# synnada-ai/datafusion-upstream

Measured on AMD Instinct MI355X. Metric: rows/sec hash-join+agg, TPC-H SF100 Q3, higher is better.
Workload: dtype int64; 1 GPU; TPC-H SF100 Q3 (3-way hash join + group-by SUM + sort), int64 keys, Decimal128(15,2) money, resident in HBM; input_rows=765043119, parallelism=1 GPU

## Files before the change

datafusion-upstream_amd/csrc/core.hip:

```cpp
#include "device_utils.h"
#include <mutex>

namespace dfgpu {

void fail(dfgpu_status code, const char* fmt, ...) {
  char buf[1024]; va_list ap; va_start(ap, fmt); vsnprintf(buf, sizeof buf, fmt, ap); va_end(ap);
  throw Error(code, buf);
}

struct CtxRefs { std::atomic<int64_t> n{1}; };
static std::mutex g_mu;
static std::vector<std::pair<dfgpu_ctx*, CtxRefs*>> g_ctx;
static CtxRefs* refs_of(dfgpu_ctx* c) { std::lock_guard<std::mutex> l(g_mu); for (auto& p : g_ctx) if (p.first == c) return p.second; return nullptr; }
static void ctx_unref(dfgpu_ctx* c) {
  CtxRefs* r = refs_of(c);
  if (!r || r->n.fetch_sub(1) != 1) return;
  { std::lock_guard<std::mutex> l(g_mu); for (size_t i = 0; i < g_ctx.size(); i++) if (g_ctx[i].first == c) { g_ctx.erase(g_ctx.begin() + i); break; } }
  (void)hipSetDevice(c->device);
  (void)hipStreamSynchronize(c->stream);
  if (c->free_blocks) { for (auto& b : *c->free_blocks) (void)hipFree(b.second); delete c->free_blocks; }
  delete c->alloc_mu;
  if (c->d_flags) (void)hipFree(c->d_flags);
  if (c->d_scratch64) (void)hipFree(c->d_scratch64);
  if (c->h_pinned) (void)hipHostFree(c->h_pinned);
  for (auto& sp : c->spans) if (sp.start) { (void)hipEventDestroy(sp.start); (void)hipEventDestroy(sp.stop); }
  if (c->copy_stream) { (void)hipStreamSynchronize(c->copy_stream); (void)hipStreamDestroy(c->copy_stream); }
  if (c->own_stream) (void)hipStreamDestroy(c->stream);
  delete r; delete c;
}

static size_t size_class(size_t bytes) {
  size_t n = 256;
  while (n < bytes) { size_t m = n + n / 2; if (m >= bytes && n >= 512) return m; n <<= 1; }
  return n;
}
Buffer::~Buffer() {
  if (owned && ptr && ctx) {
    { std::lock_guard<std::mutex> l(*ctx->alloc_mu); ctx->free_blocks->emplace_back(bytes, ptr); ctx->cached_bytes += bytes; ctx->live_bytes -= bytes; }
// ... 52 lines not shown
  struct Restore { dfgpu_ctx* c; int v; ~Restore() { c->defer_flag_checks = v; } } r{ctx, saved};
  check_flags(ctx, what.c_str());
}
void check_flags(dfgpu_ctx* ctx, const char* what) {
  if (ctx->defer_flag_checks > 0) { if (!ctx->flags_pending) ctx->flags_what = what; else if (ctx->flags_what.find(what) == std::string::npos) ctx->flags_what += std::string(", ") + what; ctx->flags_pending = true; return; }
  uint32_t f = 0;
  ctx->count_sync((std::string("sync:flags:") + what).c_str());
  fetch_to_pinned(ctx, 63, ctx->d_flags, 4);
  f = *(uint32_t*)(ctx->h_pinned + 63);
  if (!f) return;
  HIP_CHECK(hipMemsetAsync(ctx->d_flags, 0, 4, ctx->stream));
  if (f & DFGPU_FLAG_DIV_ZERO) fail(DFGPU_EXECUTION, "Arrow error: Divide by zero error (%s)", what);
  if (f & DFGPU_FLAG_OVERFLOW) fail(DFGPU_EXECUTION, "Arrow error: Arithmetic overflow (%s)", what);
  if (f & DFGPU_FLAG_CAST) fail(DFGPU_EXECUTION, "Arrow error: Cast error: value out of range (%s)", what);
  if (f & DFGPU_FLAG_OOB) fail(DFGPU_EXECUTION, "Arrow error: index out of bounds (%s)", what);
  if (f & DFGPU_FLAG_STALLED) fail(DFGPU_INTERNAL, "a workgroup gave up waiting for the tile counts of the workgroups in front of it; the result of that sort is not valid (%s; option sort_onesweep_rows=0 selects the three-launch passes)", what);
  fail(DFGPU_INTERNAL, "kernel raised flag %u (%s)", f, what);
}
__global__ void __launch_bounds__(512) k_post_words(const uint32_t* src, int nwords, uint32_t* h_dst, unsigned long long* h_seq, unsigned long long seq) {
  const int i = threadIdx.x;
  if (i < nwords) __hip_atomic_store(h_dst + i, src[i], __ATOMIC_RELAXED, __HIP_MEMORY_SCOPE_SYSTEM);
  __threadfence_system();
  __syncthreads();
  if (i == 0) __hip_atomic_store(h_seq, seq, __ATOMIC_RELEASE, __HIP_MEMORY_SCOPE_SYSTEM);
}
void fetch_to_pinned(dfgpu_ctx* ctx, int h_word, const void* d_src, size_t bytes) {
  if (bytes == 0 || (bytes & 3) || h_word < 0 || (size_t)h_word * 8 + bytes > (size_t)dfgpu_ctx::MAIL_WORDS * 8) fail(DFGPU_INTERNAL, "fetch_to_pinned: %zu bytes at word %d", bytes, h_word);
  if (!ctx->mailbox_readback) {
    HIP_CHECK(hipMemcpyAsync(ctx->h_pinned + h_word, d_src, bytes, hipMemcpyDeviceToHost, ctx->stream));
    HIP_CHECK(hipStreamSynchronize(ctx->stream));
    return;
// ... 269 lines not shown
  { "agg_partitioned_force", OPT_BOOL(agg_partitioned_force) },
  { "agg_partitioned_min_rows", OPT_INT(agg_partitioned_min_rows) },
  { "agg_pack_estimate_min_rows", OPT_INT(agg_pack_estimate_min_rows) },
  { "agg_preaggregate_distinct", OPT_READ(pa_last_distinct) },
  { "agg_spill_state_bytes", OPT_INT(agg_spill_state_bytes) },
  { "agg_spill_ranges", OPT_RANGE(agg_spill_ranges, 1, 4096) },
  { "sort_packed_keys", OPT_BOOL(sort_packed_keys) },
  { "sort_packed_min_rows", OPT_MIN(sort_packed_min_rows, 2) },
  { "sort_estimate_ranges", OPT_BOOL(sort_estimate_ranges) },
  { "sort_topk_words_min_rows", OPT_MIN(sort_topk_words_min_rows, 2) },
  { "sort_one_block_max_rows", OPT_MIN(sort_one_block_max_rows, 0) },
  { "sort_onesweep_min_rows", OPT_MIN(sort_onesweep_min_rows, 2) },
  { "sort_onesweep_rows", OPT_GET(sort_onesweep_rows), [](dfgpu_ctx* c, int64_t v) { c->sort_onesweep_rows = v == 16 ? 16 : v > 0 ? 8 : 0; } },
  { "sort_onesweep_fused_finish", OPT_BOOL(sort_onesweep_fused_finish) },
  { "sort_fused_small_passes", OPT_BOOL(sort_fused_small_passes) },
  { "sort_spill_bytes", OPT_INT(sort_spill_bytes) },
  { "sort_spill_ranges", OPT_RANGE(sort_spill_ranges, 1, 4096) },
  { "spm_merge_rows", OPT_GET(spm_merge_rows), [](dfgpu_ctx* c, int64_t v) { if (v < 0) fail(DFGPU_INVALID_ARGUMENT, "spm_merge_rows: >= 0"); c->spm_merge_rows = v; } },
  { "memory_limit", OPT_INT(memory_limit) },
  { "live_bytes", OPT_READ(live_bytes) },
  { "cached_bytes", OPT_READ(cached_bytes) },
  { "trim_cache", nullptr, [](dfgpu_ctx* c, int64_t) {
      HIP_CHECK(hipStreamSynchronize(c->stream));
      std::lock_guard<std::mutex> l(*c->alloc_mu); for (auto& x : *c->free_blocks) (void)hipFree(x.second); c->free_blocks->clear(); c->cached_bytes = 0; } },
  { "mailbox_readback", OPT_BOOL(mailbox_readback) },
  { "collect_metrics", OPT_BOOL(collect_metrics) },
  { "defer_flag_checks", OPT_GET(defer_flag_checks), [](dfgpu_ctx* c, int64_t v) {
      if (v) c->defer_flag_checks++;
      else { if (c->defer_flag_checks > 0) c->defer_flag_checks--; if (c->defer_flag_checks == 0) flush_flags(c); } } },
};
// ... 410 lines not shown
```

datafusion-upstream_amd/csrc/device_utils.h:

```cpp
#pragma once
#include "dfgpu_internal.h"

namespace dfgpu {

using i128 = __int128;
using u128 = unsigned __int128;

constexpr int WAVE = 64;
constexpr int BLOCK = 256;

__host__ __device__ inline uint64_t mix64(uint64_t x) {
  x += 0x9e3779b97f4a7c15ULL;
  x = (x ^ (x >> 30)) * 0xbf58476d1ce4e5b9ULL;
  x = (x ^ (x >> 27)) * 0x94d049bb133111ebULL;
  return x ^ (x >> 31);
}
__host__ __device__ inline uint64_t combine_hashes(uint64_t l, uint64_t r) { return ((uint64_t)(17 * 37) + l) * 37 + r; }

__device__ inline bool bit_get(const uint64_t* w, int64_t i) { return (w[i >> 6] >> (i & 63)) & 1; }
__device__ inline bool valid_at(const uint64_t* w, int64_t i) { return w == nullptr || bit_get(w, i); }

__device__ inline int lane_id() { return threadIdx.x & 63; }
__device__ inline uint64_t lanemask_lt() { return (1ull << lane_id()) - 1ull; }
__device__ inline uint64_t ballot64(bool p) { return __ballot(p); }
// ... 6 lines not shown
#pragma unroll
  for (int d = 32; d > 0; d >>= 1) v += __shfl_xor(v, d, 64);
  return v;
}
template <typename T> __device__ inline T block_exclusive_sum(T v, T* lds, T* total) {
  T inc = wave_inclusive_sum(v);
  int w = threadIdx.x >> 6;
  __syncthreads();
  if (lane_id() == 63) lds[w] = inc;
  __syncthreads();
  T base = 0, tot = 0;
#pragma unroll
  for (int i = 0; i < BLOCK / WAVE; i++) { T x = lds[i]; if (i < w) base += x; tot += x; }
  *total = tot;
  return base + inc - v;
}

__device__ inline int64_t key_at(const void* keys, int32_t key_type, int64_t i) {
  switch (key_type) {
    case DFGPU_INT8: return ((const int8_t*)keys)[i];
    case DFGPU_INT16: return ((const int16_t*)keys)[i];
    case DFGPU_INT32: case DFGPU_DATE32: return ((const int32_t*)keys)[i];
    case DFGPU_INT64: return ((const int64_t*)keys)[i];
    case DFGPU_UINT8: return ((const uint8_t*)keys)[i];
    case DFGPU_UINT16: return ((const uint16_t*)keys)[i];
    case DFGPU_UINT32: return ((const uint32_t*)keys)[i];
    default: return (int64_t)((const uint64_t*)keys)[i];
  }
}
__device__ inline bool cell_resolve(const ColView& c, int64_t i, int64_t* row) {
// ... 68 lines not shown
```

datafusion-upstream_amd/csrc/dfgpu_internal.h:

```cpp
#pragma once
#include <hip/hip_runtime.h>
#include <atomic>
#include <cstdarg>
#include <cstdint>
#include <cstdio>
#include <cstring>
#include <memory>
#include <mutex>
#include <stdexcept>
#include <string>
#include <vector>
#include "../../include/dfgpu.h"

namespace dfgpu {

struct Error : std::exception {
  dfgpu_status code; std::string msg;
  Error(dfgpu_status c, std::string m) : code(c), msg(std::move(m)) {}
  const char* what() const noexcept override { return msg.c_str(); }
};
[[noreturn]] void fail(dfgpu_status code, const char* fmt, ...);

#define HIP_CHECK(expr)                                                                         \
  do { hipError_t e_ = (expr);                                                                  \
// ... 41 lines not shown
  uint32_t* d_flags = nullptr;
  uint64_t* d_scratch64 = nullptr;
  uint64_t* h_pinned = nullptr;
  static constexpr int MAIL_SEQ = 384, MAIL_WORDS = 256, PINNED_WORDS = 512;
  bool mailbox_readback = true; uint64_t mail_seq = 0;
  int num_cus = 256;
  std::mutex* alloc_mu = nullptr;
  std::vector<std::pair<size_t, void*>>* free_blocks = nullptr;
  size_t cached_bytes = 0, live_bytes = 0;
  int64_t sort_packed_min_rows = 1 << 20;
  int64_t sort_topk_words_min_rows = 1 << 23;
  int64_t sort_one_block_max_rows = 8192;
  int64_t sort_onesweep_min_rows = 1 << 20;
  bool sort_onesweep_fused_finish = true;
  int sort_onesweep_rows = 16;
  bool sort_fused_small_passes = true;
  bool sort_estimate_ranges = true;
  int64_t spm_merge_rows = (int64_t)1 << 25;
  int64_t sort_spill_bytes = 0, sort_spill_ranges = 16;
  int64_t agg_spill_state_bytes = 0, agg_spill_ranges = 16;
  int64_t memory_limit = 0;
  bool collect_metrics = false;
  struct Span { hipEvent_t start = nullptr, stop = nullptr; };
  std::vector<Span> spans;
  std::mutex span_mu;
  bool profile = false; std::string profile_only;
  std::vector<std::pair<std::string, int64_t>> sync_counts;
  void count_sync(const char* why) { if (!profile) return; for (auto& kv : sync_counts) if (kv.first == why) { kv.second++; return; } sync_counts.emplace_back(why, 1); }
  struct ProfRec { const char* name; hipEvent_t start, stop; };
  std::vector<ProfRec> prof;
// ... 88 lines not shown
struct KeySet { int32_t n; ColView c[MAX_KEYS]; };
struct DenseCol { const void* keys; const uint64_t* key_valid; const uint32_t* canon; const uint64_t* dict_valid; int64_t dict_len; uint32_t n_ids, stride; int32_t key_type; };
struct DenseCols { int32_t n; DenseCol c[MAX_KEYS]; };
struct DeferredIds {
  int kind = 0;
  DenseCols dc{}; int32_t key_type = 0; BufferPtr mask, dense_map; std::vector<BufferPtr> keep;
  BufferPtr heads, prefix; uint32_t base = 0;
};
void materialize_ids(dfgpu_ctx* ctx, const dfgpu_array* ids);
KeySet make_keyset(const dfgpu_array* const* cols, int32_t n);

BufferPtr effective_mask(dfgpu_ctx* ctx, const dfgpu_array* mask, int64_t expect_len);

void exclusive_scan_u32(dfgpu_ctx* ctx, const uint32_t* in, uint64_t* out, int64_t n, uint64_t* d_total );
void exclusive_scan_u32_inplace32(dfgpu_ctx* ctx, uint32_t* data, int64_t n, uint64_t* d_total);

dfgpu_array* take_impl(dfgpu_ctx* ctx, const dfgpu_array* values, const void* idx, int idx_width, const uint64_t* idx_validity, int64_t n_out);
dfgpu_array* mask_to_indices_impl(dfgpu_ctx* ctx, const uint64_t* bits, int64_t n);
dfgpu_array* mask_to_indices_checked(dfgpu_ctx* ctx, const uint64_t* bits, int64_t n, int check_slot, uint64_t* check_value);
dfgpu_array* mask_to_indices_uncounted(dfgpu_ctx* ctx, const uint64_t* bits, int64_t n, uint64_t* d_count = nullptr);
int64_t count_set_bits(dfgpu_ctx* ctx, const uint64_t* bits, int64_t n);
inline const uint64_t* row_selection_words(dfgpu_ctx* ctx, int64_t n) { return ctx->row_selection && ctx->row_selection_len == n ? (const uint64_t*)ctx->row_selection->ptr : nullptr; }

void launch_iota_u32(dfgpu_ctx* ctx, uint32_t* out, int64_t n, uint32_t start);
void launch_set_bits_prefix(dfgpu_ctx* ctx, uint64_t* bits, int64_t m);

void hash_keys_device(dfgpu_ctx* ctx, const dfgpu_array* const* cols, int32_t k, uint64_t seed, uint64_t* out);

void radix_sort_pairs_u32(dfgpu_ctx* ctx, uint32_t* keys, uint32_t* vals, int64_t n, int bits);

struct KernelTimer {
  dfgpu_ctx* c; int idx = -1;
  KernelTimer(dfgpu_ctx* ctx, const char* name) : c(ctx) {
    if (!c->profile || (!c->profile_only.empty() && c->profile_only != name)) return;
// ... 25 lines not shown
```

datafusion-upstream_amd/csrc/groups.hip:

```cpp
#include "device_utils.h"
#include <algorithm>

namespace dfgpu {
constexpr uint64_t G_EMPTY = ~0ull;
constexpr uint32_t G_NEW = 0x80000000u;
constexpr uint32_t G_NONE = 0xFFFFFFFFu;
constexpr uint64_t GROUP_SEED = 0x5851f42d4c957f2dULL;
}
using namespace dfgpu;

enum class GroupRep : uint8_t { NONE, RUNS, PRIMITIVE, DENSE, DIRECT_MAP, HASHED };

struct dfgpu_groups {
  dfgpu_ctx* ctx = nullptr; int32_t nkeys = 0;
  int64_t n_groups = 0;
  GroupRep rep = GroupRep::NONE;
  std::vector<dfgpu_array*> keys;
  int64_t size_hint = 0;
  std::vector<dfgpu_array*> lazy_src; dfgpu_array* lazy_rows = nullptr;
  BufferPtr pslots; uint64_t pcap = 0; bool prim_banned = false;
  uint64_t capacity = 0; BufferPtr slots, first_row;
  BufferPtr ghash; int64_t ghash_cap = 0;
  bool canon_mode = false;
  struct Canon { dfgpu_array* dict = nullptr; BufferPtr ids; int64_t n_ids = 0; };
// ... 475 lines not shown
  if (!ctx->group_run_detection || ctx->force_hash_collisions || mk || g->capacity != 0 || !(g->n_groups == 0 || g->rep == GroupRep::RUNS) || !run_key_type(k0) ||
      (g->n_groups && logical_type(k0) != g->keys[0]->type)) return false;
  KernelTimer kt_(ctx, "k_groups_runs");
  BufferPtr heads = alloc_buffer(ctx, bitmap_bytes(n));
  zero_scratch(ctx);
  int w = type_width(k0->type);
  const void* prev = g->n_groups ? (const void*)((const char*)g->keys[0]->values->ptr + (size_t)(g->n_groups - 1) * w) : nullptr;
  dim3 grid(grid_for(n, BLOCK)), block(BLOCK);
#define RUNS(T) do { if (nkeys == 1) hipLaunchKernelGGL((k_run_heads1<T>), dim3(grid_for(n, BLOCK * 4)), block, 0, ctx->stream, (const T*)k0->values->ptr, n, (const T*)prev, (uint64_t*)heads->ptr, (unsigned long long*)(ctx->d_scratch64 + 2)); \
                     else hipLaunchKernelGGL((k_run_heads<T>), grid, block, 0, ctx->stream, bk, n, (const T*)prev, (uint64_t*)heads->ptr, (unsigned long long*)(ctx->d_scratch64 + 2)); } while (0)
  switch (k0->type) {
    case DFGPU_INT8: RUNS(int8_t); break; case DFGPU_INT16: RUNS(int16_t); break; case DFGPU_INT32: case DFGPU_DATE32: RUNS(int32_t); break; case DFGPU_INT64: RUNS(int64_t); break;
    case DFGPU_UINT8: RUNS(uint8_t); break; case DFGPU_UINT16: RUNS(uint16_t); break; case DFGPU_UINT32: RUNS(uint32_t); break; default: RUNS(uint64_t); break; }
#undef RUNS
  KERNEL_CHECK();
  ArrayHolder firsts(mask_to_indices_checked(ctx, (const uint64_t*)heads->ptr, n, 2, nullptr));
  if (!firsts.get()) return false;
  int64_t n_new = firsts.get()->length;
  if (g->n_groups + n_new >= (int64_t)G_NEW) fail(DFGPU_RESOURCES_EXHAUSTED, "more than 2^31 groups");
  int64_t nw = (n + 63) / 64;
  BufferPtr prefix = alloc_buffer(ctx, (size_t)nw * 4);
  hipLaunchKernelGGL(k_popc_words_g, dim3(grid_for(nw, BLOCK)), block, 0, ctx->stream, (const uint64_t*)heads->ptr, nw, (uint32_t*)prefix->ptr);
  exclusive_scan_u32_inplace32(ctx, (uint32_t*)prefix->ptr, nw, nullptr);
  if (allow_deferred && n >= (1 << 20)) {
    auto d = std::make_shared<DeferredIds>(); d->kind = 1; d->heads = heads; d->prefix = prefix; d->base = (uint32_t)g->n_groups; ids->deferred_ids = d;
  } else hipLaunchKernelGGL(k_run_ids, grid, block, 0, ctx->stream, (const uint64_t*)heads->ptr, (const uint32_t*)prefix->ptr, n, (uint32_t)g->n_groups, (uint32_t*)ids->values->ptr);
  KERNEL_CHECK();
  if (n_new && g->n_groups == 0 && ctx->group_lazy_keys && n_new >= (1 << 16)) {
    for (int c = 0; c < nkeys; c++) { g->lazy_src.push_back(const_cast<dfgpu_array*>(cols[c])); dfgpu_array_retain(g->lazy_src.back()); }
    g->lazy_rows = firsts.release();
  } else if (n_new) groups_append_keys(ctx, g, cols, nkeys, firsts.get(), n_new);
  g->n_groups += n_new; g->rep = GroupRep::RUNS;
  return true;
}
static bool prim_key_type(const dfgpu_array* a) { return a && (a->type == DFGPU_INT64 || a->type == DFGPU_UINT64 || a->type == DFGPU_INT32 || a->type == DFGPU_UINT32 || a->type == DFGPU_DATE32) && !a->validity; }
static void prim_rebuild(dfgpu_ctx* ctx, dfgpu_groups* g, uint64_t cap, bool key4) {
  g->pslots = alloc_buffer(ctx, (size_t)cap * sizeof(PSlot)); g->pcap = cap; HIP_CHECK(hipMemsetAsync(g->pslots->ptr, 0xFF, (size_t)cap * sizeof(PSlot), ctx->stream));
  if (!g->n_groups) return;
// ... 285 lines not shown
```

datafusion-upstream_amd/csrc/join.hip:

```cpp
#include "join_table.h"

namespace dfgpu {
constexpr uint64_t SLOT_EMPTY = ~0ull;
constexpr uint32_t NO_SLOT = 0xFFFFFFFFu;
}
using namespace dfgpu;


namespace dfgpu {

__device__ inline bool row_selected(const uint64_t* mask, int64_t i) { return mask == nullptr || bit_get(mask, i); }

__global__ void __launch_bounds__(BLOCK) k_join_build(KeySet ks, int64_t n, const uint64_t* mask, int null_eq, int force_zero,
                                                      uint64_t* slots, uint32_t* slot_count, uint64_t cap_mask, uint32_t* row_slot,
                                                      unsigned long long* counters ) {
  int64_t i = (int64_t)blockIdx.x * BLOCK + threadIdx.x;
  if (i >= n) return;
  uint32_t my_slot = NO_SLOT;
  if (row_selected(mask, i)) {
    bool any_null; uint64_t h = keyset_hash(ks, i, 0, &any_null);
    if (force_zero) h = 0;
    if (!any_null || null_eq) {
      uint64_t tag = h >> 32, s = h & cap_mask, mine = (tag << 32) | (uint64_t)i;
      for (uint64_t step = 0; step <= cap_mask; step++) {
// ... 568 lines not shown
  else {
    t->bitmap = alloc_buffer(ctx, bitmap_bytes((int64_t)range)); t->mem += (int64_t)bitmap_bytes((int64_t)range);
    HIP_CHECK(hipMemsetAsync(t->bitmap->ptr, t->rank_identity ? 0xFF : 0, bitmap_bytes((int64_t)range), ctx->stream));
  }
  if (!t->rank_identity) {
    if (mk && !runs && n <= 0xFFFFFFF0ll) {
      t->sel_rows = mask_to_indices_uncounted(ctx, mk, n, ctx->d_scratch64 + 15); t->mem += t->sel_rows->length * 4;
      DFGPU_INT_KEY_DISPATCH(key0->type, hipLaunchKernelGGL((k_key_setbits_rows<T>), dim3(grid_for(n, BLOCK, ctx->num_cus * 16)), dim3(BLOCK), 0, ctx->stream, (const T*)kv, (const uint32_t*)t->sel_rows->values->ptr,
                                                            (const unsigned long long*)(ctx->d_scratch64 + 15), (int64_t)lo, (uint64_t*)t->bitmap->ptr));
    } else {
      DFGPU_INT_KEY_DISPATCH(key0->type, hipLaunchKernelGGL((k_key_setbits_masked<T>), dim3(grid_for(n, BLOCK)), dim3(BLOCK), 0, ctx->stream, (const T*)kv, mk, n, (int64_t)lo, (uint64_t*)t->bitmap->ptr));
      if (mk) { t->sel_rows = mask_to_indices_impl(ctx, mk, n); t->mem += t->sel_rows->length * 4; }
    }
    KERNEL_CHECK();
    t->rank_prefix = alloc_buffer(ctx, (size_t)nw * 4);
    hipLaunchKernelGGL(k_popc_words, dim3(grid_for(nw, BLOCK)), dim3(BLOCK), 0, ctx->stream, (const uint64_t*)t->bitmap->ptr, nw, (uint32_t*)t->rank_prefix->ptr);
    exclusive_scan_u32_inplace32(ctx, (uint32_t*)t->rank_prefix->ptr, nw, nullptr);
    KERNEL_CHECK();
    t->mem += nw * 4;
  }
  return true;
}

template <typename T>
__global__ void __launch_bounds__(BLOCK) k_key_minmax_masked(const T* keys, const uint64_t* valid, const uint64_t* mask, int64_t n, long long* mn, long long* mx, const uint32_t* rows = nullptr, const unsigned long long* d_count = nullptr) {
  long long lo = INT64_MAX, hi = INT64_MIN;
  if (rows) {
    const int64_t m = (int64_t)*d_count;
    for (int64_t j = (int64_t)blockIdx.x * BLOCK + threadIdx.x; j < m; j += (int64_t)gridDim.x * BLOCK) { const int64_t i = rows[j]; if (valid_at(valid, i)) { long long v = (long long)keys[i]; lo = v < lo ? v : lo; hi = v > hi ? v : hi; } }
  } else
  for (int64_t i = (int64_t)blockIdx.x * BLOCK + threadIdx.x; i < n; i += (int64_t)gridDim.x * BLOCK)
    if (row_selected(mask, i) && valid_at(valid, i)) { long long v = (long long)keys[i]; lo = v < lo ? v : lo; hi = v > hi ? v : hi; }
// ... 45 lines not shown
      DFGPU_INT_KEY_DISPATCH(key0->type, hipLaunchKernelGGL((k_key_gather_minmax<T>), dim3(grid_for(n, BLOCK * 4, ctx->num_cus * 4)), dim3(BLOCK), 0, ctx->stream, (const T*)key0->values->ptr, rl, dcount, (T*)ck->ptr,
                                                            w, w + 1)); });
    lo = mm[0]; hi = mm[1];
  } else selected_key_range(ctx, t, "sync:rank_index_range", &lo, &hi);
  t->have_minmax = true; t->sel_min = lo; t->sel_max = hi;
  if (lo > hi) return false;
  const uint64_t range = (uint64_t)hi - (uint64_t)lo + 1;
  if (range == 0 || range > (1ull << 32) || range > (uint64_t)n * 256 + 65536) return false;
  const int64_t nw = (int64_t)((range + 63) / 64);
  BufferPtr bitmap = alloc_buffer(ctx, bitmap_bytes((int64_t)range));
  HIP_CHECK(hipMemsetAsync(bitmap->ptr, 0, bitmap_bytes((int64_t)range), ctx->stream));
  HIP_CHECK(hipMemsetAsync(ctx->d_scratch64 + 6, 0, 8, ctx->stream));
  DFGPU_INT_KEY_DISPATCH(key0->type, hipLaunchKernelGGL((k_key_setbits_unique<T>), dim3(lgrid), dim3(BLOCK), 0, ctx->stream, (const T*)key0->values->ptr, mk, rl, dcount, n, (int64_t)lo, (uint64_t*)bitmap->ptr,
                                                        (unsigned long long*)(ctx->d_scratch64 + 6), (const T*)ckp));
  BufferPtr prefix = alloc_buffer(ctx, (size_t)nw * 4);
  hipLaunchKernelGGL(k_popc_words, dim3(grid_for(nw, BLOCK)), dim3(BLOCK), 0, ctx->stream, (const uint64_t*)bitmap->ptr, nw, (uint32_t*)prefix->ptr);
  exclusive_scan_u32_inplace32(ctx, (uint32_t*)prefix->ptr, nw, ctx->d_scratch64 + 7);
  KERNEL_CHECK();
  const uint64_t* hsc = read_scratch_range(ctx, 6, 2);
  ctx->count_sync("sync:rank_index_unique");
  if (hsc[0] != 0) return false;
  const int64_t nsel = (int64_t)hsc[1];
  ArrayHolder rows(new_fixed(ctx, DFGPU_UINT32, nsel));
  DFGPU_INT_KEY_DISPATCH(key0->type, hipLaunchKernelGGL((k_rank_rows<T>), dim3(lgrid), dim3(BLOCK), 0, ctx->stream, (const T*)key0->values->ptr, mk, rl, dcount, n, (int64_t)lo, (const uint64_t*)bitmap->ptr,
                                                        (const uint32_t*)prefix->ptr, (uint32_t*)rows.get()->values->ptr, (const T*)ckp));
  KERNEL_CHECK();
  t->key_min = lo; t->range = range; t->rep = JoinRep::RANK; t->unique = true; t->rank_identity = false;
  t->bitmap = bitmap; t->rank_prefix = prefix; t->sel_rows = rows.release();
  t->mem += (int64_t)bitmap_bytes((int64_t)range) + nw * 4 + nsel * 4;
  return true;
}
void selected_key_range(dfgpu_ctx* ctx, const dfgpu_join_table* t, const char* sync, long long* lo, long long* hi) {
// ... 368 lines not shown
```

datafusion-upstream_amd/csrc/scan.hip:

```cpp
#include "device_utils.h"

namespace dfgpu {

constexpr int SCAN_ITEMS = 8;
constexpr int SCAN_TILE = BLOCK * SCAN_ITEMS;

__global__ void __launch_bounds__(BLOCK) k_scan_block_sums(const uint32_t* in, int64_t n, uint64_t* block_sums) {
  int64_t base = (int64_t)blockIdx.x * SCAN_TILE + (int64_t)threadIdx.x * SCAN_ITEMS;
  uint64_t s = 0;
#pragma unroll
  for (int k = 0; k < SCAN_ITEMS; k++) if (base + k < n) s += in[base + k];
  __shared__ uint64_t lds[4];
  uint64_t tot; (void)block_exclusive_sum<uint64_t>(s, lds, &tot);
  if (threadIdx.x == 0) block_sums[blockIdx.x] = tot;
}
__global__ void __launch_bounds__(BLOCK) k_scan_sums(uint64_t* sums, int64_t nb, uint64_t* d_total) {
  __shared__ uint64_t lds[4];
  uint64_t carry = 0;
  for (int64_t b0 = 0; b0 < nb; b0 += BLOCK) {
    int64_t i = b0 + threadIdx.x;
    uint64_t v = i < nb ? sums[i] : 0, tot;
    uint64_t ex = block_exclusive_sum<uint64_t>(v, lds, &tot);
    if (i < nb) sums[i] = carry + ex;
    carry += tot;
// ... 20 lines not shown
  for (int64_t t0 = 0; t0 < n; t0 += SCAN_TILE) {
    int64_t base = t0 + (int64_t)threadIdx.x * SCAN_ITEMS;
    uint32_t v[SCAN_ITEMS]; uint64_t s = 0;
#pragma unroll
    for (int k = 0; k < SCAN_ITEMS; k++) { v[k] = base + k < n ? in[base + k] : 0; s += v[k]; }
    uint64_t tot; uint64_t ex = block_exclusive_sum<uint64_t>(s, lds, &tot) + carry;
#pragma unroll
    for (int k = 0; k < SCAN_ITEMS; k++) { if (base + k < n) out[base + k] = (OUT)ex; ex += v[k]; }
    carry += tot;
    __syncthreads();
  }
  if (threadIdx.x == 0 && d_total) *d_total = carry;
}
constexpr int64_t SCAN_SMALL_MAX = 8 * SCAN_TILE;

template <typename OUT>
static void scan_impl(dfgpu_ctx* ctx, const uint32_t* in, OUT* out, int64_t n, uint64_t* d_total) {
  if (n <= 0) { if (d_total) HIP_CHECK(hipMemsetAsync(d_total, 0, 8, ctx->stream)); return; }
  if (n <= SCAN_SMALL_MAX) { hipLaunchKernelGGL((k_scan_small<OUT>), dim3(1), dim3(BLOCK), 0, ctx->stream, in, n, out, d_total); KERNEL_CHECK(); return; }
  int64_t nb = (n + SCAN_TILE - 1) / SCAN_TILE;
  BufferPtr sums = alloc_buffer(ctx, (size_t)nb * 8);
  hipLaunchKernelGGL(k_scan_block_sums, dim3((unsigned)nb), dim3(BLOCK), 0, ctx->stream, in, n, (uint64_t*)sums->ptr);
  hipLaunchKernelGGL(k_scan_sums, dim3(1), dim3(BLOCK), 0, ctx->stream, (uint64_t*)sums->ptr, nb, d_total);
  hipLaunchKernelGGL((k_scan_write<OUT>), dim3((unsigned)nb), dim3(BLOCK), 0, ctx->stream, in, n, (const uint64_t*)sums->ptr, out);
  KERNEL_CHECK();
}
void exclusive_scan_u32(dfgpu_ctx* ctx, const uint32_t* in, uint64_t* out, int64_t n, uint64_t* d_total) { scan_impl<uint64_t>(ctx, in, out, n, d_total); }
void exclusive_scan_u32_inplace32(dfgpu_ctx* ctx, uint32_t* data, int64_t n, uint64_t* d_total) { scan_impl<uint32_t>(ctx, data, data, n, d_total); }

}
```

datafusion-upstream_amd/csrc/select.hip:

```cpp
#include "device_utils.h"
#include <algorithm>

namespace dfgpu {

struct U128 { uint64_t lo, hi; };
template <int W> struct WT;
template <> struct WT<1> { using T = uint8_t; };
template <> struct WT<2> { using T = uint16_t; };
template <> struct WT<4> { using T = uint32_t; };
template <> struct WT<8> { using T = uint64_t; };
template <> struct WT<16> { using T = U128; };

__global__ void k_iota_u32(uint32_t* out, int64_t n, uint32_t start) {
  int64_t i = (int64_t)blockIdx.x * blockDim.x + threadIdx.x;
  if (i < n) out[i] = start + (uint32_t)i;
}
void launch_iota_u32(dfgpu_ctx* ctx, uint32_t* out, int64_t n, uint32_t start) {
  if (n <= 0) return;
  hipLaunchKernelGGL(k_iota_u32, dim3(grid_for(n, BLOCK)), dim3(BLOCK), 0, ctx->stream, out, n, start);
  KERNEL_CHECK();
}

__device__ inline int64_t load_index(const void* idx, int w, int64_t i) { return w == 4 ? (int64_t)((const uint32_t*)idx)[i] : (int64_t)((const uint64_t*)idx)[i]; }

// ... 144 lines not shown
  uint32_t tot; uint32_t ex = block_exclusive_sum<uint32_t>(pc, lds, &tot) + offsets[blockIdx.x];
  uint32_t wave_tot = wave_sum(pc);
  if (wave_tot == 0) return;
  if (wave_tot <= 8 * WAVE) {
    uint32_t row0 = (uint32_t)(w * 64);
    while (word) { out[ex++] = row0 + (uint32_t)__builtin_ctzll(word); word &= word - 1; }
  } else {
    int64_t wave_w0 = w - lane;
    for (int k = 0; k < WAVE; k++) {
      uint64_t m = __shfl(word, k, 64); uint32_t p = __shfl(ex, k, 64);
      if (m == 0) continue;
      if ((m >> lane) & 1) out[p + __popcll(m & lanemask_lt())] = (uint32_t)((wave_w0 + k) * 64 + lane);
    }
  }
}
dfgpu_array* mask_to_indices_impl(dfgpu_ctx* ctx, const uint64_t* bits, int64_t n) { return mask_to_indices_checked(ctx, bits, n, -1, nullptr); }
dfgpu_array* mask_to_indices_checked(dfgpu_ctx* ctx, const uint64_t* bits, int64_t n, int check_slot, uint64_t* check_value) {
  int64_t nw = (n + 63) / 64, nb = (nw + SEL_WORDS - 1) / SEL_WORDS;
  if (n == 0) { if (check_slot >= 0) { uint64_t v = read_scratch(ctx, check_slot); if (check_value) *check_value = v; if (v) return nullptr; } return new_fixed(ctx, DFGPU_UINT32, 0); }
  BufferPtr counts = alloc_buffer(ctx, (size_t)nb * 4);
  KernelTimer kt_(ctx, "k_sel_count+scan+write");
  hipLaunchKernelGGL(k_sel_count, dim3((unsigned)nb), dim3(BLOCK), 0, ctx->stream, bits, n, (uint32_t*)counts->ptr);
  exclusive_scan_u32_inplace32(ctx, (uint32_t*)counts->ptr, nb, ctx->d_scratch64 + 60);
  int64_t total;
  if (check_slot >= 0 && check_slot < 60) {
    const uint64_t* w = read_scratch_range(ctx, check_slot, 61 - check_slot);
    if (check_value) *check_value = w[0];
    if (w[0]) return nullptr;
    total = (int64_t)w[60 - check_slot];
  } else total = (int64_t)read_scratch(ctx, 60);
  ArrayHolder h(new_fixed(ctx, DFGPU_UINT32, total));
  if (total) hipLaunchKernelGGL(k_sel_write, dim3((unsigned)nb), dim3(BLOCK), 0, ctx->stream, bits, n, (const uint32_t*)counts->ptr, (uint32_t*)h.get()->values->ptr);
  h.get()->identity = total == n;
  { OrderStats st; st.sorted = true; st.repeats = false; st.exact = false; st.lo = 0; st.hi = n - 1; order_stats_set(h.get(), st); }
  KERNEL_CHECK();
  return h.release();
}


dfgpu_array* mask_to_indices_uncounted(dfgpu_ctx* ctx, const uint64_t* bits, int64_t n, uint64_t* d_count) {
  int64_t nw = (n + 63) / 64, nb = (nw + SEL_WORDS - 1) / SEL_WORDS;
  ArrayHolder h(new_fixed(ctx, DFGPU_UINT32, n));
  if (n == 0) { if (d_count) HIP_CHECK(hipMemsetAsync(d_count, 0, 8, ctx->stream)); return h.release(); }
  BufferPtr counts = alloc_buffer(ctx, (size_t)nb * 4);
  KernelTimer kt_(ctx, "k_sel_count+scan+write");
  hipLaunchKernelGGL(k_sel_count, dim3((unsigned)nb), dim3(BLOCK), 0, ctx->stream, bits, n, (uint32_t*)counts->ptr);
  exclusive_scan_u32_inplace32(ctx, (uint32_t*)counts->ptr, nb, d_count);
  hipLaunchKernelGGL(k_sel_write, dim3((unsigned)nb), dim3(BLOCK), 0, ctx->stream, bits, n, (const uint32_t*)counts->ptr, (uint32_t*)h.get()->values->ptr);
  KERNEL_CHECK();
  return h.release();
}

struct TakeCols { int32_t n; const void* src[8]; void* dst[8]; int32_t width[8]; };
template <typename IT>
__global__ void __launch_bounds__(BLOCK) k_take_multi_plain(TakeCols tc, const IT* idx, int64_t m, int64_t n_src, uint32_t* flags) {
  const int64_t base = (int64_t)blockIdx.x * BLOCK * TAKE_ROWS + threadIdx.x;
  int64_t j[TAKE_ROWS]; bool oob = false;
#pragma unroll
// ... 175 lines not shown
```

Before: 267.0 billion rows/s.

## Add single-pass decoupled-lookback prefix scan for scans and bitmap selection

```diff
diff --git a/datafusion-upstream_amd/csrc/core.hip b/datafusion-upstream_amd/csrc/core.hip
--- a/datafusion-upstream_amd/csrc/core.hip
+++ b/datafusion-upstream_amd/csrc/core.hip
@@ -22,6 +22,7 @@
   delete c->alloc_mu;
   if (c->d_flags) (void)hipFree(c->d_flags);
   if (c->d_scratch64) (void)hipFree(c->d_scratch64);
+  if (c->d_lookback) (void)hipFree(c->d_lookback);
   if (c->h_pinned) (void)hipHostFree(c->h_pinned);
   for (auto& sp : c->spans) if (sp.start) { (void)hipEventDestroy(sp.start); (void)hipEventDestroy(sp.stop); }
   if (c->copy_stream) { (void)hipStreamSynchronize(c->copy_stream); (void)hipStreamDestroy(c->copy_stream); }
@@ -104,7 +105,7 @@
   if (f & DFGPU_FLAG_OVERFLOW) fail(DFGPU_EXECUTION, "Arrow error: Arithmetic overflow (%s)", what);
   if (f & DFGPU_FLAG_CAST) fail(DFGPU_EXECUTION, "Arrow error: Cast error: value out of range (%s)", what);
   if (f & DFGPU_FLAG_OOB) fail(DFGPU_EXECUTION, "Arrow error: index out of bounds (%s)", what);
-  if (f & DFGPU_FLAG_STALLED) fail(DFGPU_INTERNAL, "a workgroup gave up waiting for the tile counts of the workgroups in front of it; the result of that sort is not valid (%s; option sort_onesweep_rows=0 selects the three-launch passes)", what);
+  if (f & DFGPU_FLAG_STALLED) fail(DFGPU_INTERNAL, "a workgroup gave up waiting for the tile sums of the workgroups in front of it; the result of that one-launch sort pass or prefix sum is not valid (%s; options sort_onesweep_rows=0 and scan_single_pass=0 select the multi-launch paths)", what);
   fail(DFGPU_INTERNAL, "kernel raised flag %u (%s)", f, what);
 }
 __global__ void __launch_bounds__(512) k_post_words(const uint32_t* src, int nwords, uint32_t* h_dst, unsigned long long* h_seq, unsigned long long seq) {
@@ -404,6 +405,7 @@
   { "sort_onesweep_rows", OPT_GET(sort_onesweep_rows), [](dfgpu_ctx* c, int64_t v) { c->sort_onesweep_rows = v == 16 ? 16 : v > 0 ? 8 : 0; } },
   { "sort_onesweep_fused_finish", OPT_BOOL(sort_onesweep_fused_finish) },
   { "sort_fused_small_passes", OPT_BOOL(sort_fused_small_passes) },
+  { "scan_single_pass", OPT_BOOL(scan_single_pass) },
   { "sort_spill_bytes", OPT_INT(sort_spill_bytes) },
   { "sort_spill_ranges", OPT_RANGE(sort_spill_ranges, 1, 4096) },
   { "spm_merge_rows", OPT_GET(spm_merge_rows), [](dfgpu_ctx* c, int64_t v) { if (v < 0) fail(DFGPU_INVALID_ARGUMENT, "spm_merge_rows: >= 0"); c->spm_merge_rows = v; } },
diff --git a/datafusion-upstream_amd/csrc/device_utils.h b/datafusion-upstream_amd/csrc/device_utils.h
--- a/datafusion-upstream_amd/csrc/device_utils.h
+++ b/datafusion-upstream_amd/csrc/device_utils.h
@@ -44,6 +44,37 @@
   for (int i = 0; i < BLOCK / WAVE; i++) { T x = lds[i]; if (i < w) base += x; tot += x; }
   *total = tot;
   return base + inc - v;
+}
+
+constexpr uint64_t LB_AGG = 1ull << 62, LB_PREFIX = 2ull << 62, LB_VAL = LB_AGG - 1ull;
+constexpr int LB_LOOK = 4;
+constexpr int LB_HEAD = 2;
+__device__ inline uint64_t lookback_exclusive(uint64_t* status, int64_t t, uint64_t agg, uint32_t* flags) {
+  const int lane = lane_id();
+  if (t == 0) { if (lane == 0) __hip_atomic_store(status, agg | LB_PREFIX, __ATOMIC_RELAXED, __HIP_MEMORY_SCOPE_AGENT); return 0; }
+  if (lane == 0) __hip_atomic_store(status + t, agg | LB_AGG, __ATOMIC_RELAXED, __HIP_MEMORY_SCOPE_AGENT);
+  uint64_t acc = 0; int64_t tt = t - 1; uint32_t idle = 0; bool done = false;
+  while (!done) {
+    uint64_t x[LB_LOOK];
+#pragma unroll
+    for (int k = 0; k < LB_LOOK; k++) { const int64_t i = tt - (k * WAVE + lane); x[k] = i >= 0 ? __hip_atomic_load(status + i, __ATOMIC_RELAXED, __HIP_MEMORY_SCOPE_AGENT) : LB_PREFIX; }
+    int used = 0; bool open = true;
+#pragma unroll
+    for (int k = 0; k < LB_LOOK; k++) if (open) {
+      const uint32_t st = (uint32_t)(x[k] >> 62);
+      const uint64_t un = ballot64(st == 0), pf = ballot64(st == 2);
+      const int fu = un ? __builtin_ctzll(un) : WAVE, fp = pf ? __builtin_ctzll(pf) : WAVE;
+      const int take = fp < fu ? fp + 1 : fu;
+      if (lane < take) acc += x[k] & LB_VAL;
+      used += take;
+      if (fp < fu) { done = true; open = false; } else if (fu < WAVE) open = false;
+    }
+    tt -= used;
+    if (!done) { if (used == 0) { __builtin_amdgcn_s_sleep(2); if (++idle > (1u << 21)) { if (lane == 0) atomicOr(flags, DFGPU_FLAG_STALLED); done = true; } } else idle = 0; }
+  }
+  const uint64_t excl = wave_sum(acc);
+  if (lane == 0) __hip_atomic_store(status + t, (excl + agg) | LB_PREFIX, __ATOMIC_RELAXED, __HIP_MEMORY_SCOPE_AGENT);
+  return excl;
 }
 
 __device__ inline int64_t key_at(const void* keys, int32_t key_type, int64_t i) {
diff --git a/datafusion-upstream_amd/csrc/dfgpu_internal.h b/datafusion-upstream_amd/csrc/dfgpu_internal.h
--- a/datafusion-upstream_amd/csrc/dfgpu_internal.h
+++ b/datafusion-upstream_amd/csrc/dfgpu_internal.h
@@ -79,6 +79,8 @@
   int64_t sort_onesweep_min_rows = 1 << 20;
   bool sort_onesweep_fused_finish = true;
   int sort_onesweep_rows = 16;
+  bool scan_single_pass = true;
+  uint64_t* d_lookback = nullptr; size_t lookback_next = 0; std::mutex lookback_mu;
   bool sort_fused_small_passes = true;
   bool sort_estimate_ranges = true;
   int64_t spm_merge_rows = (int64_t)1 << 25;
@@ -197,10 +199,12 @@
 
 void exclusive_scan_u32(dfgpu_ctx* ctx, const uint32_t* in, uint64_t* out, int64_t n, uint64_t* d_total );
 void exclusive_scan_u32_inplace32(dfgpu_ctx* ctx, uint32_t* data, int64_t n, uint64_t* d_total);
+uint64_t* lookback_words(dfgpu_ctx* ctx, int64_t tiles, BufferPtr* own);
 
 dfgpu_array* take_impl(dfgpu_ctx* ctx, const dfgpu_array* values, const void* idx, int idx_width, const uint64_t* idx_validity, int64_t n_out);
 dfgpu_array* mask_to_indices_impl(dfgpu_ctx* ctx, const uint64_t* bits, int64_t n);
-dfgpu_array* mask_to_indices_checked(dfgpu_ctx* ctx, const uint64_t* bits, int64_t n, int check_slot, uint64_t* check_value);
+dfgpu_array* mask_to_indices_checked(dfgpu_ctx* ctx, const uint64_t* bits, int64_t n, int check_slot, uint64_t* check_value, uint32_t* word_prefix = nullptr);
+void bitmap_rank_prefix(dfgpu_ctx* ctx, const uint64_t* words, int64_t nw, uint32_t* prefix, uint64_t* d_total);
 dfgpu_array* mask_to_indices_uncounted(dfgpu_ctx* ctx, const uint64_t* bits, int64_t n, uint64_t* d_count = nullptr);
 int64_t count_set_bits(dfgpu_ctx* ctx, const uint64_t* bits, int64_t n);
 inline const uint64_t* row_selection_words(dfgpu_ctx* ctx, int64_t n) { return ctx->row_selection && ctx->row_selection_len == n ? (const uint64_t*)ctx->row_selection->ptr : nullptr; }
diff --git a/datafusion-upstream_amd/csrc/groups.hip b/datafusion-upstream_amd/csrc/groups.hip
--- a/datafusion-upstream_amd/csrc/groups.hip
+++ b/datafusion-upstream_amd/csrc/groups.hip
@@ -513,14 +513,16 @@
     case DFGPU_UINT8: RUNS(uint8_t); break; case DFGPU_UINT16: RUNS(uint16_t); break; case DFGPU_UINT32: RUNS(uint32_t); break; default: RUNS(uint64_t); break; }
 #undef RUNS
   KERNEL_CHECK();
-  ArrayHolder firsts(mask_to_indices_checked(ctx, (const uint64_t*)heads->ptr, n, 2, nullptr));
+  int64_t nw = (n + 63) / 64;
+  BufferPtr prefix = alloc_buffer(ctx, (size_t)nw * 4);
+  ArrayHolder firsts(mask_to_indices_checked(ctx, (const uint64_t*)heads->ptr, n, 2, nullptr, ctx->scan_single_pass ? (uint32_t*)prefix->ptr : nullptr));
   if (!firsts.get()) return false;
   int64_t n_new = firsts.get()->length;
   if (g->n_groups + n_new >= (int64_t)G_NEW) fail(DFGPU_RESOURCES_EXHAUSTED, "more than 2^31 groups");
-  int64_t nw = (n + 63) / 64;
-  BufferPtr prefix = alloc_buffer(ctx, (size_t)nw * 4);
-  hipLaunchKernelGGL(k_popc_words_g, dim3(grid_for(nw, BLOCK)), block, 0, ctx->stream, (const uint64_t*)heads->ptr, nw, (uint32_t*)prefix->ptr);
-  exclusive_scan_u32_inplace32(ctx, (uint32_t*)prefix->ptr, nw, nullptr);
+  if (!ctx->scan_single_pass) {
+    hipLaunchKernelGGL(k_popc_words_g, dim3(grid_for(nw, BLOCK)), block, 0, ctx->stream, (const uint64_t*)heads->ptr, nw, (uint32_t*)prefix->ptr);
+    exclusive_scan_u32_inplace32(ctx, (uint32_t*)prefix->ptr, nw, nullptr);
+  }
   if (allow_deferred && n >= (1 << 20)) {
     auto d = std::make_shared<DeferredIds>(); d->kind = 1; d->heads = heads; d->prefix = prefix; d->base = (uint32_t)g->n_groups; ids->deferred_ids = d;
   } else hipLaunchKernelGGL(k_run_ids, grid, block, 0, ctx->stream, (const uint64_t*)heads->ptr, (const uint32_t*)prefix->ptr, n, (uint32_t)g->n_groups, (uint32_t*)ids->values->ptr);
diff --git a/datafusion-upstream_amd/csrc/join.hip b/datafusion-upstream_amd/csrc/join.hip
--- a/datafusion-upstream_amd/csrc/join.hip
+++ b/datafusion-upstream_amd/csrc/join.hip
@@ -606,8 +606,11 @@
     }
     KERNEL_CHECK();
     t->rank_prefix = alloc_buffer(ctx, (size_t)nw * 4);
-    hipLaunchKernelGGL(k_popc_words, dim3(grid_for(nw, BLOCK)), dim3(BLOCK), 0, ctx->stream, (const uint64_t*)t->bitmap->ptr, nw, (uint32_t*)t->rank_prefix->ptr);
-    exclusive_scan_u32_inplace32(ctx, (uint32_t*)t->rank_prefix->ptr, nw, nullptr);
+    if (ctx->scan_single_pass) bitmap_rank_prefix(ctx, (const uint64_t*)t->bitmap->ptr, nw, (uint32_t*)t->rank_prefix->ptr, nullptr);
+    else {
+      hipLaunchKernelGGL(k_popc_words, dim3(grid_for(nw, BLOCK)), dim3(BLOCK), 0, ctx->stream, (const uint64_t*)t->bitmap->ptr, nw, (uint32_t*)t->rank_prefix->ptr);
+      exclusive_scan_u32_inplace32(ctx, (uint32_t*)t->rank_prefix->ptr, nw, nullptr);
+    }
     KERNEL_CHECK();
     t->mem += nw * 4;
   }
@@ -683,8 +686,11 @@
   DFGPU_INT_KEY_DISPATCH(key0->type, hipLaunchKernelGGL((k_key_setbits_unique<T>), dim3(lgrid), dim3(BLOCK), 0, ctx->stream, (const T*)key0->values->ptr, mk, rl, dcount, n, (int64_t)lo, (uint64_t*)bitmap->ptr,
                                                         (unsigned long long*)(ctx->d_scratch64 + 6), (const T*)ckp));
   BufferPtr prefix = alloc_buffer(ctx, (size_t)nw * 4);
-  hipLaunchKernelGGL(k_popc_words, dim3(grid_for(nw, BLOCK)), dim3(BLOCK), 0, ctx->stream, (const uint64_t*)bitmap->ptr, nw, (uint32_t*)prefix->ptr);
-  exclusive_scan_u32_inplace32(ctx, (uint32_t*)prefix->ptr, nw, ctx->d_scratch64 + 7);
+  if (ctx->scan_single_pass) bitmap_rank_prefix(ctx, (const uint64_t*)bitmap->ptr, nw, (uint32_t*)prefix->ptr, ctx->d_scratch64 + 7);
+  else {
+    hipLaunchKernelGGL(k_popc_words, dim3(grid_for(nw, BLOCK)), dim3(BLOCK), 0, ctx->stream, (const uint64_t*)bitmap->ptr, nw, (uint32_t*)prefix->ptr);
+    exclusive_scan_u32_inplace32(ctx, (uint32_t*)prefix->ptr, nw, ctx->d_scratch64 + 7);
+  }
   KERNEL_CHECK();
   const uint64_t* hsc = read_scratch_range(ctx, 6, 2);
   ctx->count_sync("sync:rank_index_unique");
diff --git a/datafusion-upstream_amd/csrc/scan.hip b/datafusion-upstream_amd/csrc/scan.hip
--- a/datafusion-upstream_amd/csrc/scan.hip
+++ b/datafusion-upstream_amd/csrc/scan.hip
@@ -58,10 +58,78 @@
 }
 constexpr int64_t SCAN_SMALL_MAX = 8 * SCAN_TILE;
 
+constexpr int OP_ROUNDS = 4, OP_WAVE_ELEMS = WAVE * 4 * OP_ROUNDS, OP_TILE = (BLOCK / WAVE) * OP_WAVE_ELEMS;
+template <typename OUT>
+__global__ void __launch_bounds__(BLOCK) k_scan_onepass(const uint32_t* in, int64_t n, OUT* out, uint64_t* d_total, uint64_t* lb , uint32_t* flags) {
+  __shared__ uint64_t wtot[BLOCK / WAVE]; __shared__ uint64_t base_sh; __shared__ uint32_t tile_sh;
+  if (threadIdx.x == 0) tile_sh = atomicAdd((uint32_t*)lb, 1u);
+  __syncthreads();
+  const int64_t t = tile_sh; const int lane = lane_id(), wave = threadIdx.x >> 6;
+  const int64_t e0 = t * OP_TILE + (int64_t)wave * OP_WAVE_ELEMS + lane * 4;
+  const bool whole = (t + 1) * OP_TILE <= n;
+  const bool vin = whole && (((uintptr_t)in) & 15) == 0, vout = whole && sizeof(OUT) == 4 && (((uintptr_t)out) & 15) == 0;
+  uint32_t v[OP_ROUNDS][4];
+#pragma unroll
+  for (int r = 0; r < OP_ROUNDS; r++) {
+    const int64_t i = e0 + r * (WAVE * 4);
+    if (vin) { const uint4 q = *(const uint4*)(in + i); v[r][0] = q.x; v[r][1] = q.y; v[r][2] = q.z; v[r][3] = q.w; }
+    else {
+#pragma unroll
+      for (int j = 0; j < 4; j++) v[r][j] = i + j < n ? in[i + j] : 0;
+    }
+  }
+  uint64_t ex[OP_ROUNDS], run = 0;
+#pragma unroll
+  for (int r = 0; r < OP_ROUNDS; r++) {
+    const uint64_t s = (uint64_t)v[r][0] + v[r][1] + v[r][2] + v[r][3], inc = wave_inclusive_sum(s);
+    ex[r] = run + inc - s; run += __shfl(inc, WAVE - 1, 64);
+  }
+  if (lane == 0) wtot[wave] = run;
+  __syncthreads();
+  uint64_t wbase = 0, ttot = 0;
+#pragma unroll
+  for (int w = 0; w < BLOCK / WAVE; w++) { const uint64_t x = wtot[w]; if (w < wave) wbase += x; ttot += x; }
+  if (wave == 0) { const uint64_t e = lookback_exclusive(lb + LB_HEAD, t, ttot, flags); if (lane == 0) base_sh = e; }
+  __syncthreads();
+  const uint64_t tbase = base_sh;
+  if (d_total && threadIdx.x == 0 && t == (int64_t)gridDim.x - 1) *d_total = tbase + ttot;
+#pragma unroll
+  for (int r = 0; r < OP_ROUNDS; r++) {
+    const int64_t i = e0 + r * (WAVE * 4);
+    uint64_t e = tbase + wbase + ex[r];
+    if (vout) { uint4 q; q.x = (uint32_t)e; e += v[r][0]; q.y = (uint32_t)e; e += v[r][1]; q.z = (uint32_t)e; e += v[r][2]; q.w = (uint32_t)e; *(uint4*)((uint32_t*)out + i) = q; }
+    else {
+#pragma unroll
+      for (int j = 0; j < 4; j++) { if (i + j < n) out[i + j] = (OUT)e; e += v[r][j]; }
+    }
+  }
+}
+
+constexpr size_t LB_BLOCK_WORDS = (size_t)1 << 17;
+uint64_t* lookback_words(dfgpu_ctx* ctx, int64_t tiles, BufferPtr* own) {
+  const size_t words = ((size_t)tiles + LB_HEAD + 1) & ~(size_t)1;
+  if (words > LB_BLOCK_WORDS) {
+    *own = alloc_buffer(ctx, words * 8);
+    HIP_CHECK(hipMemsetAsync((*own)->ptr, 0, words * 8, ctx->stream));
+    return (uint64_t*)(*own)->ptr;
+  }
+  std::lock_guard<std::mutex> l(ctx->lookback_mu);
+  if (!ctx->d_lookback) { HIP_CHECK(hipMalloc((void**)&ctx->d_lookback, LB_BLOCK_WORDS * 8)); ctx->lookback_next = LB_BLOCK_WORDS; }
+  if (ctx->lookback_next + words > LB_BLOCK_WORDS) { HIP_CHECK(hipMemsetAsync(ctx->d_lookback, 0, LB_BLOCK_WORDS * 8, ctx->stream)); ctx->lookback_next = 0; }
+  uint64_t* p = ctx->d_lookback + ctx->lookback_next; ctx->lookback_next += words;
+  return p;
+}
+
 template <typename OUT>
 static void scan_impl(dfgpu_ctx* ctx, const uint32_t* in, OUT* out, int64_t n, uint64_t* d_total) {
   if (n <= 0) { if (d_total) HIP_CHECK(hipMemsetAsync(d_total, 0, 8, ctx->stream)); return; }
   if (n <= SCAN_SMALL_MAX) { hipLaunchKernelGGL((k_scan_small<OUT>), dim3(1), dim3(BLOCK), 0, ctx->stream, in, n, out, d_total); KERNEL_CHECK(); return; }
+  if (ctx->scan_single_pass) {
+    const int64_t nt = (n + OP_TILE - 1) / OP_TILE; BufferPtr own;
+    uint64_t* lb = lookback_words(ctx, nt, &own);
+    hipLaunchKernelGGL((k_scan_onepass<OUT>), dim3(grid_for(nt, 1)), dim3(BLOCK), 0, ctx->stream, in, n, out, d_total, lb, ctx->d_flags);
+    KERNEL_CHECK(); return;
+  }
   int64_t nb = (n + SCAN_TILE - 1) / SCAN_TILE;
   BufferPtr sums = alloc_buffer(ctx, (size_t)nb * 8);
   hipLaunchKernelGGL(k_scan_block_sums, dim3((unsigned)nb), dim3(BLOCK), 0, ctx->stream, in, n, (uint64_t*)sums->ptr);
diff --git a/datafusion-upstream_amd/csrc/select.hip b/datafusion-upstream_amd/csrc/select.hip
--- a/datafusion-upstream_amd/csrc/select.hip
+++ b/datafusion-upstream_amd/csrc/select.hip
@@ -182,10 +182,97 @@
     }
   }
 }
+constexpr int BT_ROUNDS = 8, BT_WAVE_WORDS = WAVE * BT_ROUNDS, BT_WORDS = (BLOCK / WAVE) * BT_WAVE_WORDS;
+template <bool LB, bool IDX, bool PFX>
+__global__ void __launch_bounds__(BLOCK) k_bits_onepass(const uint64_t* bits, int64_t n, uint32_t* tile_off, uint32_t* out_idx, uint32_t* out_pfx, uint64_t* d_total,
+                                                        uint64_t* lb , uint32_t* flags) {
+  __shared__ uint32_t wtot[BLOCK / WAVE]; __shared__ uint64_t base_sh; __shared__ uint32_t tile_sh;
+  int64_t t = blockIdx.x;
+  if (LB) { if (threadIdx.x == 0) tile_sh = atomicAdd((uint32_t*)lb, 1u); __syncthreads(); t = tile_sh; }
+  const int lane = lane_id(), wave = threadIdx.x >> 6;
+  const int64_t nw = (n + 63) >> 6, w0 = t * BT_WORDS + (int64_t)wave * BT_WAVE_WORDS;
+  uint64_t word[BT_ROUNDS];
+#pragma unroll
+  for (int r = 0; r < BT_ROUNDS; r++) { const int64_t w = w0 + r * WAVE + lane; word[r] = w < nw ? bits[w] : 0ull; if (w == nw - 1 && (n & 63)) word[r] &= (1ull << (n & 63)) - 1ull; }
+  uint32_t ex[BT_ROUNDS], seg[BT_ROUNDS], run = 0;
+#pragma unroll
+  for (int r = 0; r < BT_ROUNDS; r++) {
+    const uint32_t pc = (uint32_t)__popcll(word[r]), inc = wave_inclusive_sum(pc);
+    ex[r] = run + inc - pc; seg[r] = (uint32_t)__builtin_amdgcn_readlane((int)inc, WAVE - 1); run += seg[r];
+  }
+  if (lane == 0) wtot[wave] = run;
+  __syncthreads();
+  uint32_t wbase = 0, ttot = 0;
+#pragma unroll
+  for (int w = 0; w < BLOCK / WAVE; w++) { const uint32_t x = wtot[w]; if (w < wave) wbase += x; ttot += x; }
+  uint32_t base;
+  if (LB) {
+    if (wave == 0) { const uint64_t e = lookback_exclusive(lb + LB_HEAD, t, (uint64_t)ttot, flags); if (lane == 0) base_sh = e; }
+    __syncthreads();
+    const uint64_t tb = base_sh;
+    if (!IDX && tile_off && threadIdx.x == 0) tile_off[t] = (uint32_t)tb;
+    if (d_total && threadIdx.x == 0 && t == (int64_t)gridDim.x - 1) *d_total = tb + ttot;
+    base = (uint32_t)tb + wbase;
+  } else base = tile_off[t] + wbase;
+  if (PFX) {
+#pragma unroll
+    for (int r = 0; r < BT_ROUNDS; r++) { const int64_t w = w0 + r * WAVE + lane; if (w < nw) out_pfx[w] = base + ex[r]; }
+  }
+  if (IDX) {
+#pragma unroll
+    for (int r = 0; r < BT_ROUNDS; r++) {
+      if (seg[r] == 0) continue;
+      const int64_t sw0 = w0 + r * WAVE;
+      uint64_t m = word[r]; uint32_t e = base + ex[r];
+      if (seg[r] <= 8 * WAVE) {
+        const uint32_t row0 = (uint32_t)((sw0 + lane) * 64);
+        while (m) { out_idx[e++] = row0 + (uint32_t)__builtin_ctzll(m); m &= m - 1; }
+      } else {
+        for (int k = 0; k < WAVE; k++) {
+          const uint64_t mk = __shfl(m, k, 64); const uint32_t p = __shfl(e, k, 64);
+          if (mk == 0) continue;
+          if ((mk >> lane) & 1) out_idx[p + __popcll(mk & lanemask_lt())] = (uint32_t)((sw0 + k) * 64 + lane);
+        }
+      }
+    }
+  }
+}
+static inline int64_t bits_tiles(int64_t n) { const int64_t nw = (n + 63) / 64; return (nw + BT_WORDS - 1) / BT_WORDS; }
+void bitmap_rank_prefix(dfgpu_ctx* ctx, const uint64_t* words, int64_t nw, uint32_t* prefix, uint64_t* d_total) {
+  if (nw <= 0) { if (d_total) HIP_CHECK(hipMemsetAsync(d_total, 0, 8, ctx->stream)); return; }
+  const int64_t nt = (nw + BT_WORDS - 1) / BT_WORDS; BufferPtr own;
+  uint64_t* lb = lookback_words(ctx, nt, &own);
+  hipLaunchKernelGGL((k_bits_onepass<true, false, true>), dim3(grid_for(nt, 1)), dim3(BLOCK), 0, ctx->stream, words, nw * 64, (uint32_t*)nullptr, (uint32_t*)nullptr, prefix, d_total, lb, ctx->d_flags);
+  KERNEL_CHECK();
+}
+static dfgpu_array* mask_to_indices_onepass(dfgpu_ctx* ctx, const uint64_t* bits, int64_t n, int check_slot, uint64_t* check_value, uint32_t* word_prefix) {
+  const int64_t nt = bits_tiles(n); BufferPtr own;
+  BufferPtr offs = alloc_buffer(ctx, (size_t)nt * 4);
+  KernelTimer kt_(ctx, "k_sel_count+scan+write");
+  uint64_t* lb = lookback_words(ctx, nt, &own);
+  if (word_prefix) hipLaunchKernelGGL((k_bits_onepass<true, false, true>), dim3(grid_for(nt, 1)), dim3(BLOCK), 0, ctx->stream, bits, n, (uint32_t*)offs->ptr, (uint32_t*)nullptr, word_prefix, ctx->d_scratch64 + 60, lb, ctx->d_flags);
+  else hipLaunchKernelGGL((k_bits_onepass<true, false, false>), dim3(grid_for(nt, 1)), dim3(BLOCK), 0, ctx->stream, bits, n, (uint32_t*)offs->ptr, (uint32_t*)nullptr, (uint32_t*)nullptr, ctx->d_scratch64 + 60, lb, ctx->d_flags);
+  KERNEL_CHECK();
+  int64_t total;
+  if (check_slot >= 0 && check_slot < 60) {
+    const uint64_t* w = read_scratch_range(ctx, check_slot, 61 - check_slot);
+    if (check_value) *check_value = w[0];
+    if (w[0]) return nullptr;
+    total = (int64_t)w[60 - check_slot];
+  } else total = (int64_t)read_scratch(ctx, 60);
+  ArrayHolder h(new_fixed(ctx, DFGPU_UINT32, total));
+  if (total) hipLaunchKernelGGL((k_bits_onepass<false, true, false>), dim3(grid_for(nt, 1)), dim3(BLOCK), 0, ctx->stream, bits, n, (uint32_t*)offs->ptr, (uint32_t*)h.get()->values->ptr, (uint32_t*)nullptr, (uint64_t*)nullptr, (uint64_t*)nullptr, ctx->d_flags);
+  h.get()->identity = total == n;
+  { OrderStats st; st.sorted = true; st.repeats = false; st.exact = false; st.lo = 0; st.hi = n - 1; order_stats_set(h.get(), st); }
+  KERNEL_CHECK();
+  return h.release();
+}
 dfgpu_array* mask_to_indices_impl(dfgpu_ctx* ctx, const uint64_t* bits, int64_t n) { return mask_to_indices_checked(ctx, bits, n, -1, nullptr); }
-dfgpu_array* mask_to_indices_checked(dfgpu_ctx* ctx, const uint64_t* bits, int64_t n, int check_slot, uint64_t* check_value) {
+dfgpu_array* mask_to_indices_checked(dfgpu_ctx* ctx, const uint64_t* bits, int64_t n, int check_slot, uint64_t* check_value, uint32_t* word_prefix) {
   int64_t nw = (n + 63) / 64, nb = (nw + SEL_WORDS - 1) / SEL_WORDS;
   if (n == 0) { if (check_slot >= 0) { uint64_t v = read_scratch(ctx, check_slot); if (check_value) *check_value = v; if (v) return nullptr; } return new_fixed(ctx, DFGPU_UINT32, 0); }
+  if (ctx->scan_single_pass) return mask_to_indices_onepass(ctx, bits, n, check_slot, check_value, word_prefix);
+  if (word_prefix) fail(DFGPU_INTERNAL, "mask_to_indices_checked: word_prefix needs scan_single_pass");
   BufferPtr counts = alloc_buffer(ctx, (size_t)nb * 4);
   KernelTimer kt_(ctx, "k_sel_count+scan+write");
   hipLaunchKernelGGL(k_sel_count, dim3((unsigned)nb), dim3(BLOCK), 0, ctx->stream, bits, n, (uint32_t*)counts->ptr);
@@ -210,6 +297,14 @@
   int64_t nw = (n + 63) / 64, nb = (nw + SEL_WORDS - 1) / SEL_WORDS;
   ArrayHolder h(new_fixed(ctx, DFGPU_UINT32, n));
   if (n == 0) { if (d_count) HIP_CHECK(hipMemsetAsync(d_count, 0, 8, ctx->stream)); return h.release(); }
+  if (ctx->scan_single_pass) {
+    KernelTimer kt_(ctx, "k_sel_count+scan+write");
+    const int64_t nt = bits_tiles(n); BufferPtr own;
+    uint64_t* lb = lookback_words(ctx, nt, &own);
+    hipLaunchKernelGGL((k_bits_onepass<true, true, false>), dim3(grid_for(nt, 1)), dim3(BLOCK), 0, ctx->stream, bits, n, (uint32_t*)nullptr, (uint32_t*)h.get()->values->ptr, (uint32_t*)nullptr, d_count, lb, ctx->d_flags);
+    KERNEL_CHECK();
+    return h.release();
+  }
   BufferPtr counts = alloc_buffer(ctx, (size_t)nb * 4);
   KernelTimer kt_(ctx, "k_sel_count+scan+write");
   hipLaunchKernelGGL(k_sel_count, dim3((unsigned)nb), dim3(BLOCK), 0, ctx->stream, bits, n, (uint32_t*)counts->ptr);
```

After: 259.0 billion rows/s. 0.97x the previous value.
